# liruiluo/VLA-Adapter

Hardware: AMD Instinct MI355X
Metric: fine-tune samples/sec (224px img + 32-tok prompt), adapter-only, fwd+bwd+AdamW (higher is better)
Workload: dtype bf16

## Files before the change

### vla_adapter_amd/csrc/elementwise.hip

```cpp
#include "gemm_epilogue.h"
#include <type_traits>

namespace {

inline unsigned nblk(long long n, int per) { return (unsigned)((n + per - 1) / per); }

__global__ void im2col_kernel(const void* __restrict__ px, bf16_t* __restrict__ out, int B, int Ctot, int c0, int H,
                              int W, int P, int ldo, int f32in) {
  const int gw = W / P, gh = H / P, KK = 3 * P * P;
  const long long total = (long long)B * gh * gw * ldo;
  for (long long i = (long long)blockIdx.x * blockDim.x + threadIdx.x; i < total; i += (long long)gridDim.x * blockDim.x) {
    const int col = i % ldo;
    const long long prow = i / ldo;
    float v = 0.f;
    if (col < KK) {
      const int c = col / (P * P), rem = col - c * P * P, py = rem / P, pxx = rem - py * P;
      const int pw = prow % gw, ph = (prow / gw) % gh, b = prow / ((long long)gw * gh);
      const long long src = (((long long)b * Ctot + c0 + c) * H + ph * P + py) * W + pw * P + pxx;
      v = f32in ? ((const float*)px)[src] : bf2f(((const bf16_t*)px)[src]);
    }
    out[i] = f2bf(v);
  }
}

__global__ void action_mask_kernel(const long long* __restrict__ labels, int* __restrict__ qidx, int* __restrict__ pos,
                                   int* __restrict__ count, int B, int L, int shift) {
  const int b = blockIdx.x, lane = threadIdx.x;
  const long long* row = labels + (long long)b * L + shift;
  const int n = L - shift;
  int base = 0;
  for (int j0 = 0; j0 < n; j0 += 64) {
    const int j = j0 + lane;
    const bool sel = j < n && row[j] != -100 && row[j] > 151386;
    const unsigned long long bal = __ballot(sel);
    const int k = base + __popcll(bal & ((1ull << lane) - 1ull));
    if (j < n) qidx[(long long)b * n + j] = sel ? k : -1;
    if (sel && k < 64) pos[b * 64 + k] = j;
    base += __popcll(bal);
  }
  if (lane == 0) count[b] = base;
  for (int k = base + lane; k < 64; k += 64) pos[b * 64 + k] = -1;
}

__global__ void embed_splice_kernel(const long long* __restrict__ ids, const unsigned char* __restrict__ am,
                                    const int* __restrict__ qidx, const bf16_t* __restrict__ table,
                                    const bf16_t* __restrict__ aq, bf16_t* __restrict__ out,
                                    unsigned char* __restrict__ mm, int B, int L, int Np, int D, int vocab) {
  const int S = L + Np;
  const int lane = threadIdx.x & 63;
  const long long r = (long long)blockIdx.x * 4 + (threadIdx.x >> 6);
  if (r >= (long long)B * S) return;
  const int b = r / S, s = r - (long long)b * S;
  if (s >= 1 && s <= Np) {
    if (lane == 0 && mm) mm[r] = 1;
    return;
  }
  const int j = s == 0 ? 0 : s - Np;
  const int qi = qidx[(long long)b * L + j];
  long long id = ids[(long long)b * L + j];
  if (id < 0 || id >= vocab) id = 0;
  const bf16_t* src = qi >= 0 ? aq + (long long)min(qi, 63) * D : table + id * D;
  bf16_t* dst = out + r * D;
  for (int e = lane * 8; e < D; e += 512) *reinterpret_cast<uint4*>(dst + e) = *reinterpret_cast<const uint4*>(src + e);
  if (lane == 0 && mm) mm[r] = am ? (am[(long long)b * L + j] != 0) : 1;
}

__global__ void action_query_grad_kernel(const bf16_t* __restrict__ dx, const int* __restrict__ pos, float* __restrict__ dq,
                                         int B, int S, int Np, int D, int row0) {
  const int k = blockIdx.x;
  for (int d = threadIdx.x; d < D; d += blockDim.x) {
    float a = 0.f;
    for (int b = 0; b < B; ++b) {
      const int j = pos[b * 64 + k];
      if (j < 0) continue;
      const int s = (j == 0 ? 0 : Np + j) - row0;
      if (s < 0) continue;
      a += bf2f(dx[((long long)b * S + s) * D + d]);
    }
    dq[k * D + d] = a;
  }
}

__global__ void gather_rows_kernel(const bf16_t* __restrict__ in, const int* __restrict__ idx, bf16_t* __restrict__ out,
                                   int n, int D, int ldi, int ldo) {
  const int lane = threadIdx.x & 63;
  const long long r = (long long)blockIdx.x * 4 + (threadIdx.x >> 6);
  if (r >= n) return;
  const int s = idx[r];
  if (s == -2) return;
  for (int e = lane * 8; e < D; e += 512) {
    uint4 v = s >= 0 ? *reinterpret_cast<const uint4*>(in + (long long)s * ldi + e) : uint4{0, 0, 0, 0};
    *reinterpret_cast<uint4*>(out + r * ldo + e) = v;
  }
}

__global__ void scatter_add_rows_kernel(const bf16_t* __restrict__ in, const int* __restrict__ idx, bf16_t* __restrict__ out,
                                        int n, int D, int ldi, int ldo) {
  const int lane = threadIdx.x & 63;
  const long long r = (long long)blockIdx.x * 4 + (threadIdx.x >> 6);
  if (r >= n) return;
  const int s = idx[r];
  if (s < 0) return;
  for (int e = lane * 8; e < D; e += 512) {
    float a[8], c[8];
    unpack8(*reinterpret_cast<const uint4*>(in + r * ldi + e), a);
    unpack8(*reinterpret_cast<const uint4*>(out + (long long)s * ldo + e), c);
#pragma unroll
    for (int k = 0; k < 8; ++k) c[k] += a[k];
    *reinterpret_cast<uint4*>(out + (long long)s * ldo + e) = pack8(c);
  }
}

enum { EW_ADD = 0, EW_GELU_F = 1, EW_GELU_B = 2, EW_RELU_B = 3 };
template <int OP>
__global__ void ew_kernel(const bf16_t* __restrict__ a, const bf16_t* __restrict__ b, bf16_t* __restrict__ y, long long n8) {
  for (long long i = (long long)blockIdx.x * blockDim.x + threadIdx.x; i < n8; i += (long long)gridDim.x * blockDim.x) {
    float fa[8], fb[8] = {0, 0, 0, 0, 0, 0, 0, 0}, o[8];
    unpack8(reinterpret_cast<const uint4*>(a)[i], fa);
    if (OP != EW_GELU_F) unpack8(reinterpret_cast<const uint4*>(b)[i], fb);
#pragma unroll
    for (int k = 0; k < 8; ++k) {
      if (OP == EW_ADD) o[k] = fa[k] + fb[k];
      else if (OP == EW_GELU_F) o[k] = gelu_erf(fa[k]);
      else if (OP == EW_GELU_B) o[k] = fa[k] * gelu_erf_grad(fb[k]);
      else o[k] = fb[k] > 0.f ? fa[k] : 0.f;
    }
    reinterpret_cast<uint4*>(y)[i] = pack8(o);
  }
}

__global__ void swiglu_bwd_kernel(const bf16_t* __restrict__ dh, const bf16_t* __restrict__ gu, bf16_t* __restrict__ dgu,
                                  long long nchunks, int I) {
  const int cpr = I / 8;
  for (long long i = (long long)blockIdx.x * blockDim.x + threadIdx.x; i < nchunks; i += (long long)gridDim.x * blockDim.x) {
    const long long m = i / cpr;
    const int c = (int)(i - m * cpr) * 8;
    const long long go = m * 2 * I + (c >> 4) * 32 + (c & 15);
    float d[8], g[8], u[8], dg[8], du[8];
    unpack8(*reinterpret_cast<const uint4*>(dh + m * I + c), d);
    unpack8(*reinterpret_cast<const uint4*>(gu + go), g);
    unpack8(*reinterpret_cast<const uint4*>(gu + go + 16), u);
#pragma unroll
    for (int k = 0; k < 8; ++k) {
      const float sg = 1.f / (1.f + __expf(-g[k]));
      du[k] = d[k] * (g[k] * sg);
      dg[k] = d[k] * u[k] * silu_grad(g[k], sg);
    }
    *reinterpret_cast<uint4*>(dgu + go) = pack8(dg);
    *reinterpret_cast<uint4*>(dgu + go + 16) = pack8(du);
  }
}

__global__ __launch_bounds__(256) void transpose_kernel(const bf16_t* __restrict__ in, bf16_t* __restrict__ out, int rows,
                                                        int cols, int ldi, int ldo, long long s_in, long long s_out) {
  __shared__ bf16_t t[64][66];
  const bf16_t* ib = in + (long long)blockIdx.z * s_in;
  bf16_t* ob = out + (long long)blockIdx.z * s_out;
  const int r0 = blockIdx.y * 64, c0 = blockIdx.x * 64;
  const int tx = threadIdx.x & 63, ty = threadIdx.x >> 6;
  for (int r = ty; r < 64; r += 4)
    t[r][tx] = (r0 + r < rows && c0 + tx < cols) ? ib[(long long)(r0 + r) * ldi + c0 + tx] : (bf16_t)0;
  __syncthreads();
  for (int c = ty; c < 64; c += 4)
    if (c0 + c < cols && r0 + tx < rows) ob[(long long)(c0 + c) * ldo + r0 + tx] = t[tx][c];
}

__global__ __launch_bounds__(256) void transpose_vec_kernel(const bf16_t* __restrict__ in, bf16_t* __restrict__ out, int rows,
                                                            int cols, int ldi, int ldo, long long s_in, long long s_out) {
  __shared__ unsigned t32[64 * 33];
  const bf16_t* ib = in + (long long)blockIdx.z * s_in;
  bf16_t* ob = out + (long long)blockIdx.z * s_out;
  const int r0 = blockIdx.y * 64, c0 = blockIdx.x * 64;
  for (int i = threadIdx.x; i < 512; i += 256) {
    const int r = i >> 3, ch = i & 7;
    uint4 v = {0u, 0u, 0u, 0u};
    if (r0 + r < rows && c0 + ch * 8 < cols) v = *reinterpret_cast<const uint4*>(ib + (long long)(r0 + r) * ldi + c0 + ch * 8);
    unsigned* d = t32 + r * 33 + ch * 4;
    d[0] = v.x; d[1] = v.y; d[2] = v.z; d[3] = v.w;
  }
  __syncthreads();
  const bf16_t* t = reinterpret_cast<const bf16_t*>(t32);
  for (int i = threadIdx.x; i < 512; i += 256) {
    const int g = i & 7, c = i >> 3;
    if (c0 + c < cols && r0 + g * 8 < rows) {
      unsigned o[4];
#pragma unroll
      for (int k = 0; k < 4; ++k)
        o[k] = (unsigned)t[(g * 8 + 2 * k) * 66 + c] | ((unsigned)t[(g * 8 + 2 * k + 1) * 66 + c] << 16);
      *reinterpret_cast<uint4*>(ob + (long long)(c0 + c) * ldo + r0 + g * 8) = uint4{o[0], o[1], o[2], o[3]};
    }
  }
}

__global__ void colsum_kernel(const bf16_t* __restrict__ x, float* __restrict__ out, int rows, int cols, int ldx, long long s_x,
                              long long s_out) {
  const int c = blockIdx.x * 256 + threadIdx.x;
  if (c >= cols) return;
  x += (long long)blockIdx.z * s_x;
  out += (long long)blockIdx.z * s_out;
  float a = 0.f;
  for (int r = 0; r < rows; ++r) a += bf2f(x[(long long)r * ldx + c]);
  atomicAdd(out + c, a);
}

template <int LPR>
__global__ __launch_bounds__(CR_THREADS) void colsum_vec_kernel(const bf16_t* __restrict__ x, float* __restrict__ out, int rows, int cols,
                                                                int ldx, long long s_x, long long s_out) {
  __shared__ float sm[CR_THREADS / 64][64];
  const int c = CR<LPR>::col();
  x += (long long)blockIdx.z * s_x;
  out += (long long)blockIdx.z * s_out;
  float a[8] = {0, 0, 0, 0, 0, 0, 0, 0};
  if (c < cols)
    for (int r = CR<LPR>::row0(); r < rows; r += CR<LPR>::GROUPS) {
      float f[8];
      unpack8(*reinterpret_cast<const uint4*>(x + (long long)r * ldx + c), f);
#pragma unroll
      for (int k = 0; k < 8; ++k) a[k] += f[k];
    }
  CR<LPR>::add(a, out, cols, sm);
}

__global__ void cast_f32_bf16_kernel(const float* __restrict__ x, bf16_t* __restrict__ y, long long n) {
  for (long long i = (long long)blockIdx.x * blockDim.x + threadIdx.x; i < n; i += (long long)gridDim.x * blockDim.x) y[i] = f2bf(x[i]);
}
__global__ void cast_bf16_f32_kernel(const bf16_t* __restrict__ x, float* __restrict__ y, long long n) {
  for (long long i = (long long)blockIdx.x * blockDim.x + threadIdx.x; i < n; i += (long long)gridDim.x * blockDim.x) y[i] = bf2f(x[i]);
}

__global__ void rope_half_kernel(bf16_t* __restrict__ x, const float* __restrict__ ct, const float* __restrict__ st, long long rows,
                                 int S, int nheads, int dh, int ldx, float sign) {
  const int half = dh / 2;
  const long long total = rows * nheads * half;
// ... 130 lines not shown
template <bool CLIP>
__global__ void adamw_vec8_kernel(uint4* __restrict__ p, const void* __restrict__ g, uint4* __restrict__ m, uint4* __restrict__ v,
                                  long long n8, float decay, float omb1, float beta2, float omb2, float bc2_sqrt, float eps,
                                  float neg_step, int g_f32, float gscale, const float* __restrict__ coef) {
  const float c = CLIP ? *coef : 1.f;
  for (long long i = (long long)blockIdx.x * blockDim.x + threadIdx.x; i < n8; i += (long long)gridDim.x * blockDim.x) {
    const uint4 pv = p[i], mv = m[i], vv = v[i];
    float gr[8];
    adamw_grad8(g, i, g_f32, gscale, gr);
    if (CLIP) {
#pragma unroll
      for (int k = 0; k < 8; ++k) gr[k] = rbf(gr[k] * c);
    }
    const unsigned pw[4] = {pv.x, pv.y, pv.z, pv.w}, mw[4] = {mv.x, mv.y, mv.z, mv.w}, vw[4] = {vv.x, vv.y, vv.z, vv.w};
    unsigned po[4], mo[4], vo[4];
#pragma unroll
    for (int k = 0; k < 4; ++k) {
      float p0 = bf_lo(pw[k]), p1 = bf_hi(pw[k]);
      float m0 = bf_lo(mw[k]), m1 = bf_hi(mw[k]);
      float v0 = bf_lo(vw[k]), v1 = bf_hi(vw[k]);
      adamw_one(p0, gr[2 * k], m0, v0, decay, omb1, beta2, omb2, bc2_sqrt, eps, neg_step);
      adamw_one(p1, gr[2 * k + 1], m1, v1, decay, omb1, beta2, omb2, bc2_sqrt, eps, neg_step);
      po[k] = pack2(p0, p1); mo[k] = pack2(m0, m1); vo[k] = pack2(v0, v1);
    }
    p[i] = uint4{po[0], po[1], po[2], po[3]};
    m[i] = uint4{mo[0], mo[1], mo[2], mo[3]};
    v[i] = uint4{vo[0], vo[1], vo[2], vo[3]};
  }
}

constexpr int GRAD_SSQ_ITERS = 8;
constexpr long long GRAD_SSQ_CHUNK = 256LL * 8 * GRAD_SSQ_ITERS;
template <bool F32>
__global__ __launch_bounds__(256) void grad_sumsq_kernel(const void* __restrict__ g, long long n, float gscale, float* __restrict__ slots) {
  typedef typename std::conditional<F32, float, bf16_t>::type T;
  __shared__ float red[4];
  const long long c0 = (long long)blockIdx.x * GRAD_SSQ_CHUNK;
  const int cnt = (int)min(GRAD_SSQ_CHUNK, n - c0), tid = threadIdx.x;
  const T* base = (const T*)g + c0;
  const int head = min(cnt, (int)(((16 - ((uintptr_t)base & 15)) & 15) / sizeof(T)));
  const int nv = (cnt - head) / 8, tail0 = head + nv * 8;
  const T* body = base + head;
  float acc = 0.f, gr[8];
  if (nv == 256 * GRAD_SSQ_ITERS) {
    float x[GRAD_SSQ_ITERS][8];
#pragma unroll
    for (int it = 0; it < GRAD_SSQ_ITERS; ++it) adamw_grad8(body, it * 256 + tid, F32, gscale, x[it]);
#pragma unroll
    for (int it = 0; it < GRAD_SSQ_ITERS; ++it)
#pragma unroll
      for (int k = 0; k < 8; ++k) acc = __builtin_fmaf(x[it][k], x[it][k], acc);
  } else {
    for (int j = tid; j < nv; j += 256) {
      adamw_grad8(body, j, F32, gscale, gr);
#pragma unroll
      for (int k = 0; k < 8; ++k) acc = __builtin_fmaf(gr[k], gr[k], acc);
    }
  }
  if (tid < head) {
    const float x = adamw_grad<F32>(F32 ? ((const float*)base)[tid] : bf2f(((const bf16_t*)base)[tid]), gscale);
    acc = __builtin_fmaf(x, x, acc);
  }
  if (tid < cnt - tail0) {
    const float x = adamw_grad<F32>(F32 ? ((const float*)base)[tail0 + tid] : bf2f(((const bf16_t*)base)[tail0 + tid]), gscale);
    acc = __builtin_fmaf(x, x, acc);
  }
  acc = wave_sum(acc);
  if ((tid & 63) == 0) red[tid >> 6] = acc;
  __syncthreads();
  if (tid == 0) slots[blockIdx.x] = ((red[0] + red[1]) + red[2]) + red[3];
}

__global__ __launch_bounds__(256) void grad_norm_finalise_kernel(const float* __restrict__ slots, long long n_slots, float max_norm,
                                                                 float* __restrict__ out) {
  __shared__ double red[256];
  const int tid = threadIdx.x;
  double s = 0.0;
  for (long long i = tid; i < n_slots; i += 256) s += (double)slots[i];
  red[tid] = s;
  __syncthreads();
  for (int o = 128; o > 0; o >>= 1) {
    if (tid < o) red[tid] += red[tid + o];
    __syncthreads();
  }
  if (tid == 0) {
    const float total = (float)sqrt(red[0]);
    const float c = (1.f / (total + 1e-6f)) * max_norm;
    out[0] = total;
    out[1] = c > 1.f ? 1.f : c;
  }
}

}

#define GRID1D(n, per) dim3(min(nblk((n), (per)), 8192u))

__global__ void image_normalize_kernel(const unsigned char* __restrict__ img, void* __restrict__ out, int B, int H, int W, int Ctot,
                                       int c0, float m0, float m1, float m2, float s0, float s1, float s2, int out_f32) {
  const long long total = (long long)B * 3 * H * W;
  for (long long i = (long long)blockIdx.x * blockDim.x + threadIdx.x; i < total; i += (long long)gridDim.x * blockDim.x) {
    const int x = (int)(i % W);
    const int y = (int)((i / W) % H);
    const int c = (int)((i / ((long long)W * H)) % 3);
    const long long b = i / ((long long)3 * W * H);
    const float t = (float)img[((b * H + y) * W + x) * 3 + c] / 255.0f;
    const float v = (t - (c == 0 ? m0 : c == 1 ? m1 : m2)) / (c == 0 ? s0 : c == 1 ? s1 : s2);
    const long long o = ((b * Ctot + c0 + c) * H + y) * W + x;
    if (out_f32) reinterpret_cast<float*>(out)[o] = v;
    else reinterpret_cast<bf16_t*>(out)[o] = f2bf(v);
  }
}

__global__ void action_tokenize_kernel(const float* __restrict__ act, const double* __restrict__ bins, long long* __restrict__ ids,
                                       long long n, int nbins, float lo, float hi, long long tokenizer_len) {
  const long long i = (long long)blockIdx.x * blockDim.x + threadIdx.x;
  if (i >= n) return;
  ids[i] = action_token_id(act[i], bins, nbins, lo, hi, tokenizer_len);
}

extern "C" int vla_im2col_patch(void* stream, const void* pixels, void* cols, int B, int Ctot, int c0, int H, int W, int P,
                                int ldo, int px_f32) {
  VLA_REQUIRE(pixels && cols && B > 0 && P > 0 && H % P == 0 && W % P == 0, "im2col: bad shape");
  VLA_REQUIRE(c0 >= 0 && c0 + 3 <= Ctot && ldo >= 3 * P * P, "im2col: channel window / ldo");
  const long long total = (long long)B * (H / P) * (W / P) * ldo;
  hipLaunchKernelGGL(im2col_kernel, GRID1D(total, 256), dim3(256), 0, (hipStream_t)stream, pixels, (bf16_t*)cols, B, Ctot, c0,
                     H, W, P, ldo, px_f32);
  VLA_CHECK_LAUNCH("im2col");
  return VLA_OK;
}

extern "C" int vla_action_mask(void* stream, const long long* labels, int* qidx, int* pos, int* count, int B, int L, int shift) {
  VLA_REQUIRE(labels && qidx && pos && count && B > 0 && L > shift && (shift == 0 || shift == 1), "action_mask: bad args");
  hipLaunchKernelGGL(action_mask_kernel, dim3(B), dim3(64), 0, (hipStream_t)stream, labels, qidx, pos, count, B, L, shift);
  VLA_CHECK_LAUNCH("action_mask");
  return VLA_OK;
}

extern "C" int vla_embed_splice(void* stream, const long long* ids, const unsigned char* attn_mask, const int* qidx,
                                const void* table, const void* action_queries, void* out, unsigned char* mm_mask, int B,
                                int L, int Np, int D, int vocab) {
  VLA_REQUIRE(ids && qidx && table && action_queries && out && B > 0 && L > 0 && Np >= 0 && D % 8 == 0 && vocab > 0,
              "embed_splice: bad args");
  VLA_REQUIRE(((((uintptr_t)table) | ((uintptr_t)action_queries) | ((uintptr_t)out)) & 15) == 0, "embed_splice: 16-B aligned table / action_queries / out");
  const long long rows = (long long)B * (L + Np);
  hipLaunchKernelGGL(embed_splice_kernel, dim3(nblk(rows, 4)), dim3(256), 0, (hipStream_t)stream, ids, attn_mask, qidx,
                     (const bf16_t*)table, (const bf16_t*)action_queries, (bf16_t*)out, mm_mask, B, L, Np, D, vocab);
  VLA_CHECK_LAUNCH("embed_splice");
  return VLA_OK;
}

extern "C" int vla_action_query_grad(void* stream, const void* dx, const int* pos, float* dq, int B, int S, int Np, int D,
                                     int row0) {
  VLA_REQUIRE(dx && pos && dq && B > 0 && S > 0 && S + row0 > Np && D > 0 && row0 >= 0, "action_query_grad: bad args");
  hipLaunchKernelGGL(action_query_grad_kernel, dim3(64), dim3(256), 0, (hipStream_t)stream, (const bf16_t*)dx, pos, dq, B, S, Np, D, row0);
  VLA_CHECK_LAUNCH("action_query_grad");
  return VLA_OK;
}

extern "C" int vla_gather_rows(void* stream, const void* in, const int* idx, void* out, int n, int D, int ldi, int ldo) {
  VLA_REQUIRE(in && idx && out && n > 0 && D % 8 == 0 && ldi % 8 == 0 && ldo % 8 == 0, "gather_rows: bad args");
  VLA_REQUIRE(((((uintptr_t)in) | ((uintptr_t)out)) & 15) == 0, "gather_rows: 16-B aligned in / out");
  hipLaunchKernelGGL(gather_rows_kernel, dim3(nblk(n, 4)), dim3(256), 0, (hipStream_t)stream, (const bf16_t*)in, idx, (bf16_t*)out, n, D, ldi, ldo);
  VLA_CHECK_LAUNCH("gather_rows");
  return VLA_OK;
}

extern "C" int vla_scatter_add_rows(void* stream, const void* in, const int* idx, void* out, int n, int D, int ldi, int ldo) {
  VLA_REQUIRE(in && idx && out && n > 0 && D % 8 == 0 && ldi % 8 == 0 && ldo % 8 == 0, "scatter_add_rows: bad args");
  VLA_REQUIRE(((((uintptr_t)in) | ((uintptr_t)out)) & 15) == 0, "scatter_add_rows: 16-B aligned in / out");
  hipLaunchKernelGGL(scatter_add_rows_kernel, dim3(nblk(n, 4)), dim3(256), 0, (hipStream_t)stream, (const bf16_t*)in, idx, (bf16_t*)out, n, D, ldi, ldo);
  VLA_CHECK_LAUNCH("scatter_add_rows");
  return VLA_OK;
}

#define EW_ENTRY(NAME, OP, NEEDB)                                                                                  \
  extern "C" int NAME(void* stream, const void* a, const void* b, void* y, long long n) {                           \
    VLA_REQUIRE(a && y && (!(NEEDB) || b) && n > 0 && n % 8 == 0, #NAME ": null / n%8");                              \
    VLA_REQUIRE(((((uintptr_t)a) | ((uintptr_t)b) | ((uintptr_t)y)) & 15) == 0, #NAME ": 16-B aligned tensors");     \
    hipLaunchKernelGGL(ew_kernel<OP>, GRID1D(n / 8, 256), dim3(256), 0, (hipStream_t)stream, (const bf16_t*)a,     \
                       (const bf16_t*)b, (bf16_t*)y, n / 8);                                                       \
    VLA_CHECK_LAUNCH(#NAME);                                                                                       \
    return VLA_OK;                                                                                                 \
  }
EW_ENTRY(vla_add_bf16, EW_ADD, 1)
EW_ENTRY(vla_gelu_bwd, EW_GELU_B, 1)
EW_ENTRY(vla_relu_bwd, EW_RELU_B, 1)
extern "C" int vla_gelu_fwd(void* stream, const void* x, void* y, long long n) {
  VLA_REQUIRE(x && y && n > 0 && n % 8 == 0, "gelu_fwd: null / n%8");
  VLA_REQUIRE(((((uintptr_t)x) | ((uintptr_t)y)) & 15) == 0, "gelu_fwd: 16-B aligned tensors");
  hipLaunchKernelGGL(ew_kernel<EW_GELU_F>, GRID1D(n / 8, 256), dim3(256), 0, (hipStream_t)stream, (const bf16_t*)x,
                     (const bf16_t*)nullptr, (bf16_t*)y, n / 8);
  VLA_CHECK_LAUNCH("gelu_fwd");
  return VLA_OK;
}

extern "C" int vla_swiglu_bwd(void* stream, const void* dh, const void* gu, void* dgu, int M, int I) {
  VLA_REQUIRE(dh && gu && dgu && M > 0 && I > 0 && I % 16 == 0, "swiglu_bwd: I%16");
  VLA_REQUIRE(((((uintptr_t)dh) | ((uintptr_t)gu) | ((uintptr_t)dgu)) & 15) == 0, "swiglu_bwd: 16-B aligned tensors");
  const long long nch = (long long)M * (I / 8);
  hipLaunchKernelGGL(swiglu_bwd_kernel, GRID1D(nch, 256), dim3(256), 0, (hipStream_t)stream, (const bf16_t*)dh, (const bf16_t*)gu, (bf16_t*)dgu, nch, I);
  VLA_CHECK_LAUNCH("swiglu_bwd");
  return VLA_OK;
}

extern "C" int vla_transpose_bf16(void* stream, const void* in, void* out, int rows, int cols, int ldi, int ldo, int batch,
                                  long long s_in, long long s_out) {
  VLA_REQUIRE(in && out && rows > 0 && cols > 0 && ldi >= cols && ldo >= rows && batch > 0, "transpose: bad args");
  dim3 grid((cols + 63) / 64, (rows + 63) / 64, batch);
  const bool vec = rows % 8 == 0 && cols % 8 == 0 && ldi % 8 == 0 && ldo % 8 == 0 && s_in % 8 == 0 && s_out % 8 == 0 &&
                   ((((uintptr_t)in) | ((uintptr_t)out)) & 15) == 0;
  if (vec)
    hipLaunchKernelGGL(transpose_vec_kernel, grid, dim3(256), 0, (hipStream_t)stream, (const bf16_t*)in, (bf16_t*)out, rows, cols, ldi, ldo, s_in, s_out);
  else
    hipLaunchKernelGGL(transpose_kernel, grid, dim3(256), 0, (hipStream_t)stream, (const bf16_t*)in, (bf16_t*)out, rows, cols, ldi, ldo, s_in, s_out);
  VLA_CHECK_LAUNCH("transpose");
  return VLA_OK;
}

extern "C" int vla_colsum_bf16(void* stream, const void* x, float* out, int rows, int cols, int ldx, int batch, long long s_x,
                               long long s_out) {
  VLA_REQUIRE(x && out && rows > 0 && cols > 0 && ldx >= cols && batch > 0, "colsum: bad args");
  if (cols % 8 == 0 && ldx % 8 == 0 && s_x % 8 == 0 && ((uintptr_t)x & 15) == 0) {
    CR_LAUNCH(colsum_vec_kernel, rows, cols, batch, stream, (const bf16_t*)x, out, rows, cols, ldx, s_x, s_out);
    VLA_CHECK_LAUNCH("colsum");
    return VLA_OK;
  }
  hipLaunchKernelGGL(colsum_kernel, dim3((cols + 255) / 256, 1, batch), dim3(256), 0, (hipStream_t)stream, (const bf16_t*)x, out, rows,
                     cols, ldx, s_x, s_out);
  VLA_CHECK_LAUNCH("colsum");
  return VLA_OK;
}

extern "C" int vla_cast_f32_bf16(void* stream, const float* x, void* y, long long n) {
  VLA_REQUIRE(x && y && n > 0, "cast: bad args");
  hipLaunchKernelGGL(cast_f32_bf16_kernel, GRID1D(n, 256), dim3(256), 0, (hipStream_t)stream, x, (bf16_t*)y, n);
  VLA_CHECK_LAUNCH("cast_f32_bf16");
  return VLA_OK;
}
extern "C" int vla_cast_bf16_f32(void* stream, const void* x, float* y, long long n) {
  VLA_REQUIRE(x && y && n > 0, "cast: bad args");
  hipLaunchKernelGGL(cast_bf16_f32_kernel, GRID1D(n, 256), dim3(256), 0, (hipStream_t)stream, (const bf16_t*)x, y, n);
  VLA_CHECK_LAUNCH("cast_bf16_f32");
  return VLA_OK;
}

extern "C" int vla_rope_half(void* stream, void* x, const float* cos_t, const float* sin_t, int rows, int S, int nheads, int dh,
                             int ldx, int sign) {
  VLA_REQUIRE(x && cos_t && sin_t && rows > 0 && S > 0 && nheads > 0 && dh % 2 == 0 && ldx >= nheads * dh, "rope_half: bad args");
  const long long total = (long long)rows * nheads * (dh / 2);
  hipLaunchKernelGGL(rope_half_kernel, GRID1D(total, 256), dim3(256), 0, (hipStream_t)stream, (bf16_t*)x, cos_t, sin_t, (long long)rows, S, nheads, dh, ldx, sign >= 0 ? 1.f : -1.f);
  VLA_CHECK_LAUNCH("rope_half");
  return VLA_OK;
}

extern "C" int vla_rope_interleaved(void* stream, void* x, const float* cos_t, const float* sin_t, int rows, int T, int nheads,
                                    int dh, int ldx, int mode) {
  VLA_REQUIRE(x && cos_t && sin_t && rows > 0 && T > 0 && nheads > 0 && dh % 2 == 0 && ldx >= nheads * dh, "rope_interleaved: bad args");
  const long long total = (long long)rows * nheads * (dh / 2);
  if (dh % 8 == 0 && ldx % 8 == 0 && (((uintptr_t)x | (uintptr_t)cos_t | (uintptr_t)sin_t) & 15) == 0) {
    const long long tv = (long long)rows * (nheads * dh / 8);
    hipLaunchKernelGGL(rope_inter_vec_kernel, GRID1D(tv, 256), dim3(256), 0, (hipStream_t)stream, (bf16_t*)x, cos_t, sin_t, (int)rows, T, nheads, dh, ldx, mode);
  } else
  hipLaunchKernelGGL(rope_inter_kernel, GRID1D(total, 256), dim3(256), 0, (hipStream_t)stream, (bf16_t*)x, cos_t, sin_t, (long long)rows, T, nheads, dh, ldx, mode);
  VLA_CHECK_LAUNCH("rope_interleaved");
  return VLA_OK;
}

extern "C" int vla_l1_loss(void* stream, const void* pred, const void* target, float* loss3, void* dpred, int B, int C, int Da,
                           float gscale) {
  VLA_REQUIRE(pred && target && loss3 && B > 0 && C > 0 && Da > 0, "l1_loss: bad args");
  hipLaunchKernelGGL(l1_loss_kernel, dim3(1), dim3(256), 0, (hipStream_t)stream, (const bf16_t*)pred, (const bf16_t*)target, loss3, (bf16_t*)dpred, B, C, Da, gscale);
  VLA_CHECK_LAUNCH("l1_loss");
  return VLA_OK;
}

static int adamw_launch(void* stream, void* p, const void* g, void* m, void* v, long long n, double lr, double beta1, double beta2,
                        double eps, double wd, int step, int g_f32, float gscale, const float* coef) {
  VLA_REQUIRE(p && g && m && v && n > 0 && step >= 1, "adamw: bad args");
  const double bc1 = 1.0 - pow(beta1, step), bc2 = 1.0 - pow(beta2, step);
  const float decay = (float)(1.0 - lr * wd);
  const float omb1 = (float)(1.0 - beta1), omb2 = (float)(1.0 - beta2);
  const float neg_step = (float)(-(lr / bc1));
  const float gs = gscale == 0.f ? 1.f : gscale;
  const bool aligned = ((((uintptr_t)p) | ((uintptr_t)g) | ((uintptr_t)m) | ((uintptr_t)v)) & 15) == 0;
  const long long n8 = aligned ? n / 8 : 0, done = n8 * 8;
  if (n8 > 0)
    hipLaunchKernelGGL(coef ? adamw_vec8_kernel<true> : adamw_vec8_kernel<false>, GRID1D(n8, 256), dim3(256), 0, (hipStream_t)stream,
                       (uint4*)p, g, (uint4*)m, (uint4*)v, n8, decay, omb1, (float)beta2, omb2, (float)sqrt(bc2), (float)eps, neg_step,
                       g_f32, gs, coef);
  if (done < n)
    hipLaunchKernelGGL(coef ? adamw_kernel<true> : adamw_kernel<false>, GRID1D(n - done, 256), dim3(256), 0, (hipStream_t)stream,
                       (bf16_t*)p + done, g_f32 ? (const void*)((const float*)g + done) : (const void*)((const bf16_t*)g + done),
                       (bf16_t*)m + done, (bf16_t*)v + done, n - done, decay, omb1, (float)beta2, omb2, (float)sqrt(bc2), (float)eps,
                       neg_step, g_f32, gs, coef);
  VLA_CHECK_LAUNCH("adamw");
  return VLA_OK;
}

extern "C" int vla_adamw_bf16(void* stream, void* p, const void* g, void* m, void* v, long long n, double lr, double beta1,
                              double beta2, double eps, double wd, int step, int g_f32, float gscale) {
  return adamw_launch(stream, p, g, m, v, n, lr, beta1, beta2, eps, wd, step, g_f32, gscale, nullptr);
}

extern "C" int vla_adamw_clipped_bf16(void* stream, void* p, const void* g, void* m, void* v, long long n, double lr, double beta1,
                                      double beta2, double eps, double wd, int step, int g_f32, float gscale, const float* coef) {
  VLA_REQUIRE(coef, "adamw_clipped: null coefficient");
  return adamw_launch(stream, p, g, m, v, n, lr, beta1, beta2, eps, wd, step, g_f32, gscale, coef);
}

extern "C" long long vla_grad_sumsq_slots(long long n) { return n > 0 ? (n + GRAD_SSQ_CHUNK - 1) / GRAD_SSQ_CHUNK : 0; }

extern "C" int vla_grad_sumsq(void* stream, const void* g, long long n, int g_f32, float gscale, float* slots) {
  VLA_REQUIRE(g && slots && n > 0, "grad_sumsq: bad args");
  VLA_REQUIRE(((uintptr_t)g & (g_f32 ? 3 : 1)) == 0 && ((uintptr_t)slots & 3) == 0, "grad_sumsq: misaligned pointer");
  const long long nb = vla_grad_sumsq_slots(n);
  VLA_REQUIRE(nb <= 0x7fffffffLL, "grad_sumsq: slice too long");
  const float gs = gscale == 0.f ? 1.f : gscale;
  hipLaunchKernelGGL(g_f32 ? grad_sumsq_kernel<true> : grad_sumsq_kernel<false>, dim3((unsigned)nb), dim3(256), 0, (hipStream_t)stream, g, n, gs, slots);
  VLA_CHECK_LAUNCH("grad_sumsq");
  return VLA_OK;
}

extern "C" int vla_grad_norm_finalise(void* stream, const float* slots, long long n_slots, float max_norm, float* out2) {
  VLA_REQUIRE(slots && out2 && n_slots > 0 && max_norm > 0.f, "grad_norm_finalise: bad args");
  hipLaunchKernelGGL(grad_norm_finalise_kernel, dim3(1), dim3(256), 0, (hipStream_t)stream, slots, n_slots, max_norm, out2);
  VLA_CHECK_LAUNCH("grad_norm_finalise");
  return VLA_OK;
}

extern "C" int vla_image_normalize_u8(void* stream, const void* img, void* out, int B, int H, int W, int Ctot, int c0,
                                      const float* mean3, const float* std3, int out_f32) {
  VLA_REQUIRE(img && out && mean3 && std3 && B > 0 && H > 0 && W > 0 && c0 >= 0 && c0 + 3 <= Ctot, "image_normalize: bad args");
  VLA_REQUIRE(std3[0] != 0.f && std3[1] != 0.f && std3[2] != 0.f, "image_normalize: zero std");
  const long long total = (long long)B * 3 * H * W;
  hipLaunchKernelGGL(image_normalize_kernel, GRID1D(total, 256), dim3(256), 0, (hipStream_t)stream, (const unsigned char*)img, out, B,
                     H, W, Ctot, c0, mean3[0], mean3[1], mean3[2], std3[0], std3[1], std3[2], out_f32);
  VLA_CHECK_LAUNCH("image_normalize");
  return VLA_OK;
}

extern "C" int vla_action_tokenize(void* stream, const float* actions, const double* bins, long long* ids, long long n, int nbins,
                                   float lo, float hi, long long tokenizer_len) {
  VLA_REQUIRE(actions && bins && ids && n > 0 && nbins > 1 && lo < hi, "action_tokenize: bad args");
  hipLaunchKernelGGL(action_tokenize_kernel, dim3((unsigned)((n + 255) / 256)), dim3(256), 0, (hipStream_t)stream, actions, bins, ids, n,
                     nbins, lo, hi, tokenizer_len);
  VLA_CHECK_LAUNCH("action_tokenize");
  return VLA_OK;
}


template <typename TS, typename TD>
__global__ void copy2d_kernel(const TS* __restrict__ src, TD* __restrict__ dst, long long rows, int cols, long long ld_src, long long ld_dst,
                              int src_mod, int d_group, long long d_group_stride) {
  const long long total = rows * cols;
  for (long long i = (long long)blockIdx.x * blockDim.x + threadIdx.x; i < total; i += (long long)gridDim.x * blockDim.x) {
    const long long r = i / cols;
    const int c = (int)(i - r * cols);
    const long long rs = src_mod > 0 ? r % src_mod : r;
    const long long ro = d_group > 0 ? (r / d_group) * d_group_stride + (r % d_group) * ld_dst : r * ld_dst;
    float v;
    if constexpr (sizeof(TS) == 2) v = bf2f(src[rs * ld_src + c]); else v = src[rs * ld_src + c];
    if constexpr (sizeof(TD) == 2) dst[ro + c] = f2bf(v); else dst[ro + c] = v;
  }
}

__global__ void quant_fp8_rows_kernel(const bf16_t* __restrict__ x, unsigned char* __restrict__ q, float* __restrict__ scale, int rows, int cols,
                                      long long ldx, long long ldq) {
  const int lane = threadIdx.x & 63, row = blockIdx.x * (blockDim.x >> 6) + (threadIdx.x >> 6);
  if (row >= rows) return;
  const bf16_t* xr = x + (long long)row * ldx;
  float amax = 0.f;
  for (int c = lane * 8; c < cols; c += 512) {
    const uint4 v = *reinterpret_cast<const uint4*>(xr + c);
    const unsigned w[4] = {v.x, v.y, v.z, v.w};
#pragma unroll
    for (int k = 0; k < 4; ++k) amax = fmaxf(amax, fmaxf(fabsf(bf_lo(w[k])), fabsf(bf_hi(w[k]))));
  }
  amax = wave_max(amax);
  const float inv = amax > 0.f ? __fdiv_rn(448.f, amax) : 1.f;
  if (lane == 0) scale[row] = amax > 0.f ? __fdiv_rn(amax, 448.f) : 1.f;
  unsigned char* qr = q + (long long)row * ldq;
  for (int c = lane * 8; c < cols; c += 512) {
    const uint4 v = *reinterpret_cast<const uint4*>(xr + c);
    const unsigned w[4] = {v.x, v.y, v.z, v.w};
    int lo = 0, hi = 0;
    lo = __builtin_amdgcn_cvt_pk_fp8_f32(bf_lo(w[0]) * inv, bf_hi(w[0]) * inv, lo, false);
    lo = __builtin_amdgcn_cvt_pk_fp8_f32(bf_lo(w[1]) * inv, bf_hi(w[1]) * inv, lo, true);
    hi = __builtin_amdgcn_cvt_pk_fp8_f32(bf_lo(w[2]) * inv, bf_hi(w[2]) * inv, hi, false);
    hi = __builtin_amdgcn_cvt_pk_fp8_f32(bf_lo(w[3]) * inv, bf_hi(w[3]) * inv, hi, true);
    *reinterpret_cast<uint2*>(qr + c) = uint2{(unsigned)lo, (unsigned)hi};
  }
}

extern "C" int vla_quant_fp8_rows(void* stream, const void* x, void* q, float* scale, int rows, int cols, int ldx, int ldq) {
  VLA_REQUIRE(x && q && scale && rows > 0 && cols > 0 && cols % 8 == 0 && ldx % 8 == 0 && ldx >= cols && ldq >= cols && ldq % 16 == 0 &&
                  ((((uintptr_t)x) | ((uintptr_t)q)) & 15) == 0,
              "quant_fp8_rows: cols % 8, ldx % 8, ldq % 16, 16-B aligned pointers");
  hipLaunchKernelGGL(quant_fp8_rows_kernel, dim3((rows + 3) / 4), dim3(256), 0, (hipStream_t)stream, (const bf16_t*)x, (unsigned char*)q, scale, rows,
                     cols, (long long)ldx, (long long)ldq);
  VLA_CHECK_LAUNCH("quant_fp8_rows");
  return VLA_OK;
}

__global__ void copy2d_vec_kernel(const uint4* __restrict__ src, uint4* __restrict__ dst, long long rows, long long cols16, long long ld_src16,
                                  long long ld_dst16) {
  const long long total = rows * cols16;
  for (long long i = (long long)blockIdx.x * blockDim.x + threadIdx.x; i < total; i += (long long)gridDim.x * blockDim.x) {
    const long long r = i / cols16, c = i - r * cols16;
    dst[r * ld_dst16 + c] = src[r * ld_src16 + c];
  }
}

extern "C" int vla_copy2d(void* stream, const void* src, void* dst, long long rows, int cols, long long ld_src, long long ld_dst,
                          int src_dtype, int dst_dtype, int src_mod, int d_group, long long d_group_stride) {
  VLA_REQUIRE(src && dst && rows > 0 && cols > 0 && src_mod >= 0 && d_group >= 0, "copy2d: bad args");
  VLA_REQUIRE((src_dtype == 0 || src_dtype == 1) && (dst_dtype == 0 || dst_dtype == 1), "copy2d: dtype 0 (bf16) / 1 (f32)");
  hipStream_t st = (hipStream_t)stream;
  const int esz = src_dtype == 0 ? 2 : 4, per16 = 16 / esz;
  if (src_dtype == dst_dtype && src_mod == 0 && d_group == 0 && cols % per16 == 0 && ld_src % per16 == 0 && ld_dst % per16 == 0 &&
      ((((uintptr_t)src) | ((uintptr_t)dst)) & 15) == 0) {
    const long long c16 = cols / per16;
    hipLaunchKernelGGL(copy2d_vec_kernel, GRID1D(rows * c16, 256), dim3(256), 0, st, (const uint4*)src, (uint4*)dst, rows, c16, ld_src / per16,
                       ld_dst / per16);
    VLA_CHECK_LAUNCH("copy2d");
    return VLA_OK;
  }
  const dim3 g = GRID1D(rows * cols, 256);
#define CP(TS, TD) hipLaunchKernelGGL((copy2d_kernel<TS, TD>), g, dim3(256), 0, st, (const TS*)src, (TD*)dst, rows, cols, ld_src, ld_dst, src_mod, d_group, d_group_stride)
  if (src_dtype == 0 && dst_dtype == 0) CP(bf16_t, bf16_t);
  else if (src_dtype == 1 && dst_dtype == 0) CP(float, bf16_t);
  else if (src_dtype == 0 && dst_dtype == 1) CP(bf16_t, float);
  else CP(float, float);
#undef CP
  VLA_CHECK_LAUNCH("copy2d");
  return VLA_OK;
}

__global__ void fill_zero_kernel(uint4* __restrict__ p16, long long n16, unsigned char* __restrict__ tail, int ntail) {
  const long long i0 = (long long)blockIdx.x * blockDim.x + threadIdx.x;
  for (long long i = i0; i < n16; i += (long long)gridDim.x * blockDim.x) p16[i] = uint4{0, 0, 0, 0};
  if (i0 < ntail) tail[i0] = 0;
}

extern "C" int vla_fill_zero(void* stream, void* ptr, long long nbytes) {
  VLA_REQUIRE(ptr && nbytes > 0 && ((uintptr_t)ptr & 15) == 0, "fill_zero: null / empty / not 16-B aligned");
  const long long n16 = nbytes / 16;
  hipLaunchKernelGGL(fill_zero_kernel, GRID1D(n16 > 0 ? n16 : 1, 256), dim3(256), 0, (hipStream_t)stream, (uint4*)ptr, n16,
                     (unsigned char*)ptr + n16 * 16, (int)(nbytes - n16 * 16));
  VLA_CHECK_LAUNCH("fill_zero");
  return VLA_OK;
}

__device__ __forceinline__ unsigned long long drop_hash(unsigned long long seed, unsigned long long idx) { return splitmix64_key(seed, idx); }

template <bool ADD>
__global__ void dropout_kernel(const bf16_t* __restrict__ x, bf16_t* __restrict__ y, long long rows, int cols, long long ldx, long long ldy,
                               unsigned thr, float scale, unsigned long long seed, const int* __restrict__ step) {
  const int cpr = cols >> 3;
  const long long total = rows * cpr;
  const unsigned long long sd = seed + (unsigned long long)(step ? *step : 0) * 0xD1B54A32D192ED03ull;
  for (long long i = (long long)blockIdx.x * blockDim.x + threadIdx.x; i < total; i += (long long)gridDim.x * blockDim.x) {
    const long long r = i / cpr;
    const int c = (int)(i - r * cpr) * 8;
    const unsigned long long h0 = drop_hash(sd, 2ull * (unsigned long long)i), h1 = drop_hash(sd, 2ull * (unsigned long long)i + 1);
    const uint4 xv = *reinterpret_cast<const uint4*>(x + r * ldx + c);
    const unsigned xw[4] = {xv.x, xv.y, xv.z, xv.w};
    uint4 yv = uint4{0, 0, 0, 0};
    if (ADD) yv = *reinterpret_cast<const uint4*>(y + r * ldy + c);
    unsigned yw[4] = {yv.x, yv.y, yv.z, yv.w};
#pragma unroll
    for (int k = 0; k < 4; ++k) {
      const unsigned long long h = k < 2 ? h0 : h1;
      const bool k0 = ((unsigned)(h >> (32 * (k & 1))) & 0xffffu) >= thr, k1 = ((unsigned)(h >> (32 * (k & 1) + 16)) & 0xffffu) >= thr;
      const float a = k0 ? rbf(bf_lo(xw[k]) * scale) : 0.f, b = k1 ? rbf(bf_hi(xw[k]) * scale) : 0.f;
      if (ADD) yw[k] = pack2(bf_lo(yw[k]) + a, bf_hi(yw[k]) + b);
      else yw[k] = pack2(a, b);
    }
    *reinterpret_cast<uint4*>(y + r * ldy + c) = uint4{yw[0], yw[1], yw[2], yw[3]};
  }
}

static int dropout_launch(bool add, void* stream, const void* x, void* y, long long rows, int cols, long long ldx, long long ldy, float p,
                          unsigned long long seed, const int* step) {
  VLA_REQUIRE(x && y && rows > 0 && cols > 0 && cols % 8 == 0 && ldx % 8 == 0 && ldy % 8 == 0 && (((uintptr_t)x | (uintptr_t)y) & 15) == 0,
              "dropout: null / empty / cols, row strides must be multiples of 8 and the tensors 16-B aligned");
  VLA_REQUIRE(p >= 0.f && p < 1.f, "dropout: p in [0, 1)");
  const unsigned thr = (unsigned)(p * 65536.f + 0.5f);
  const float scale = 1.f / (1.f - p);
  const long long total = rows * (cols / 8);
  if (add) hipLaunchKernelGGL(dropout_kernel<true>, GRID1D(total, 256), dim3(256), 0, (hipStream_t)stream, (const bf16_t*)x, (bf16_t*)y, rows, cols, ldx, ldy, thr, scale, seed, step);
  else hipLaunchKernelGGL(dropout_kernel<false>, GRID1D(total, 256), dim3(256), 0, (hipStream_t)stream, (const bf16_t*)x, (bf16_t*)y, rows, cols, ldx, ldy, thr, scale, seed, step);
  VLA_CHECK_LAUNCH("dropout");
  return VLA_OK;
}

extern "C" int vla_dropout_bf16(void* stream, const void* x, void* y, long long rows, int cols, long long ldx, long long ldy, float p,
                                unsigned long long seed, const int* step) {
  return dropout_launch(false, stream, x, y, rows, cols, ldx, ldy, p, seed, step);
}

extern "C" int vla_dropout_bwd_add_bf16(void* stream, const void* u, void* dx, long long rows, int cols, long long ldu, long long lddx, float p,
                                        unsigned long long seed, const int* step) {
  return dropout_launch(true, stream, u, dx, rows, cols, ldu, lddx, p, seed, step);
}

__global__ void inc_i32_kernel(int* p) { if (threadIdx.x == 0 && blockIdx.x == 0) *p += 1; }

extern "C" int vla_inc_i32(void* stream, int* ptr) {
  VLA_REQUIRE(ptr, "inc_i32: null");
  hipLaunchKernelGGL(inc_i32_kernel, dim3(1), dim3(64), 0, (hipStream_t)stream, ptr);
  VLA_CHECK_LAUNCH("inc_i32");
  return VLA_OK;
}

__global__ void head_index_prep_kernel(const int* __restrict__ pos1, const int* __restrict__ pos0, const int* __restrict__ cnt0,
                                       int* __restrict__ gather, int* __restrict__ scatter, float* __restrict__ guard,
                                       int B, int S, int Np, int row0) {
  const int i = blockIdx.x * blockDim.x + threadIdx.x;
  if (i < B * 65) {
    const int b = i / 65, k = i - b * 65;
    if (k == 64) {
      gather[i] = -2;
      scatter[i] = -1;
    } else {
      const int p = pos1[b * 64 + k];
      gather[i] = b * S + Np + p;
      const int loc = Np + p - row0;
      scatter[i] = (loc >= 0 && p >= 0) ? b * (S - row0) + loc : -1;
    }
  }
  if (i == 0 && guard) {
    bool bad = false;
    for (int b = 0; b < B; ++b) bad |= (row0 > 0) && ((cnt0[b] > 0 ? pos0[b * 64] + Np : 0) < row0);
    *guard = bad ? __int_as_float(0x7fc00000) : 0.f;
  }
}

extern "C" int vla_head_index_prep(void* stream, const int* pos1, const int* pos0, const int* cnt0, int* gather, int* scatter,
                                   float* guard, int B, int S, int Np, int row0) {
  VLA_REQUIRE(pos1 && pos0 && cnt0 && gather && scatter && B > 0 && S > row0 && row0 >= 0, "head_index_prep: bad args");
  hipLaunchKernelGGL(head_index_prep_kernel, dim3(nblk((long long)B * 65, 256)), dim3(256), 0, (hipStream_t)stream, pos1, pos0, cnt0, gather,
                     scatter, guard, B, S, Np, row0);
  VLA_CHECK_LAUNCH("head_index_prep");
  return VLA_OK;
}

__global__ void add_scalar_f32_kernel(float* __restrict__ x, const float* __restrict__ s, int n) {
  const int i = blockIdx.x * blockDim.x + threadIdx.x;
  if (i < n) x[i] += *s;
}

extern "C" int vla_add_scalar_f32(void* stream, float* x, const float* s, int n) {
  VLA_REQUIRE(x && s && n > 0, "add_scalar_f32: bad args");
  hipLaunchKernelGGL(add_scalar_f32_kernel, dim3(nblk(n, 256)), dim3(256), 0, (hipStream_t)stream, x, s, n);
  VLA_CHECK_LAUNCH("add_scalar_f32");
  return VLA_OK;
}


__global__ void embed_grad_kernel(const bf16_t* __restrict__ dx, const long long* __restrict__ ids, const int* __restrict__ qidx,
                                  bf16_t* __restrict__ gtable, int B, int L, int Np, int D, int vocab) {
  const int t = blockIdx.x, n = B * L;
  if (qidx[t] >= 0) return;
  long long id = ids[t];
  if (id < 0 || id >= vocab) id = 0;
  __shared__ int first;
  if (threadIdx.x == 0) {
    int f = 1;
    for (int u = 0; u < t && f; ++u) {
      long long iu = ids[u];
      if (iu < 0 || iu >= vocab) iu = 0;
      if (qidx[u] < 0 && iu == id) f = 0;
    }
    first = f;
  }
  __syncthreads();
// ... 394 lines not shown
```

### vla_adapter_amd/engine.py

```python
from __future__ import annotations

import contextlib
import math
import os
from dataclasses import dataclass, field
from typing import Dict, List, Optional, Tuple

import torch

from . import ops, schedule
from .ops import ACT_GELU, ACT_GELU_TANH, ACT_NONE, ACT_RELU, ACT_SWIGLU, BF16
from .schedule import Segment, capture_graph, chunks, turnaround_chunks

NUM_TOKENS = 64
IGNORE_INDEX = -100


def rup(n: int, m: int) -> int:
    return (n + m - 1) // m * m


def copy_flat(dst: torch.Tensor, src: torch.Tensor):
    n = src.numel()
    ops.copy2d(src, dst, 1, n, n, n)
# ... 1143 lines not shown
                self._query_grad()

        return (schedule.pipeline_forward(head, fch, llm_fwd, lambda: (llm.HS, self.pos1, batch["proprio"], self.Np, noise), turn_around,
                                          refresh=True)
                + schedule.pipeline_backward(head, fch, llm_bwd, lambda: self._dHS)
                + [Segment("H", head.bwd_end, None, ("end", 0))])

    def _stream_of(self, name: str, main):
        return main if name == "M" else self.side if name == "H" else self._vstreams[int(name[1:])]

    def _cap_stream(self, name: str):
        return self._cap_main if name == "M" else self._stream_of(name, None)

    def _fwd_bwd(self, batch, noise, vision: bool = True):
        self.executed_steps += 1
        if vision:
            self._vision(batch)
        torch.cuda.current_stream().wait_event(schedule.run(self._segments(batch, noise), self._stream_of)[("end", 0)])
        return self._loss3

    def capture(self, batch: Dict[str, torch.Tensor], noise: Optional[torch.Tensor] = None, warmup: int = 2,
                conservative_rows: bool = False, row0: Optional[int] = None):
        self._ensure_streams()
        self._static_batch, self._static_noise = batch, noise
        self._row0 = None
        self._vision_and_embed(batch)
        self._row0 = self.live_row0()
        if conservative_rows and not self.full_llm_backward:
            self._row0 = min(self._row0, (self.cfg.n_patches + 1) // 32 * 32)
        if row0 is not None:
            assert 0 <= int(row0) < self.S and int(row0) % 32 == 0, f"row0 {row0}: a multiple of 32 inside the sequence"
            self._row0 = int(row0)
        for _ in range(warmup):
            self.head.dirty = True
            self._fwd_bwd(batch, noise)
        torch.cuda.synchronize()
        self.head.dirty = True
        self._next_px = batch["pixel_values"].clone()
        self._px_stage = batch["pixel_values"].clone()
        self._g_vis = capture_graph(lambda: self._vision(dict(batch, pixel_values=self._px_stage)), torch.cuda.graph_pool_handle(),
                                    self.vis_stream)
        self._vis_ev = None
        self._segs = self._segments(batch, noise)
        self._graphs = schedule.capture(self._segs, {}, self._cap_stream)
        torch.cuda.synchronize()
        self._pending_lr = None
        m_fwd = [k for k, sg in enumerate(self._segs) if sg.stream == "M" and sg.signal is not None and sg.signal[0] == "f"]
        self._vis_after = m_fwd[min(len(m_fwd) - 1, max(0, int(os.environ.get("VLA_VIS_AFTER", len(m_fwd) - 4))))]
        assert self._segs[self._vis_after].signal is not None
        self._launch_vision()

    def stage_next_pixels(self, pixel_values: torch.Tensor):
        if self._px_copied is not None:
            torch.cuda.current_stream().wait_event(self._px_copied)
        self._next_px.copy_(pixel_values)

    def _launch_vision(self, after_event=None):
        V, cur = self.vis_stream, torch.cuda.current_stream()
        if after_event is not None:
            V.wait_event(after_event)
        else:
            V.wait_stream(cur)
        tl = self._timeline
        with torch.cuda.stream(V):
            if tl is not None:
                t0 = torch.cuda.Event(enable_timing=True)
                t0.record(V)
            copy_flat(self._px_stage, self._next_px)
            self._px_copied = torch.cuda.Event()
            self._px_copied.record(V)
            self._g_vis.replay()
            self._vis_ev = torch.cuda.Event(enable_timing=tl is not None)
            self._vis_ev.record(V)
            if tl is not None:
                tl.append(("V", -1, t0, self._vis_ev))

    def train_step_pipelined(self, batch, lr: float, noise=None):
        self._ensure_streams()
        loss3 = self._fwd_bwd(batch, noise)
        if self.reducer is not None:
            self.reducer.reduce_async(self.head.P.grad, 0, None)
        self.optimizer_step(lr)
        return loss3

    def train_step_graphed(self, lr: float):
        cur = torch.cuda.current_stream()
        self.executed_steps += 1
        self.flush(join=False)
        cur.wait_event(self._vis_ev)
        def after(k, seg, ev):
            if k == self._vis_after:
                self._launch_vision(ev)
        self._h_end = schedule.run(self._segs, self._stream_of, self._graphs, after=after,
                                   timeline=self._timeline)[("end", 0)]
        cur.wait_event(self._px_copied)
        if self.ga > 1:
            cur.wait_event(self._h_end)
            if not self._accum.fold():
                return self._loss3
            self._h_end = torch.cuda.Event()
            self._h_end.record(cur)
        if self.reducer is not None:
            aq_off = self.head.P.offsets["action_queries"][0]
            ev_aq = self.reducer.reduce_async(self.head.P.grad, aq_off, None)
            ev_head = self.reducer.reduce_async(self.head.P.grad, 0, aq_off, after_event=self._h_end)
            self._reduced = (ev_aq, ev_head)
        self._pending_lr = lr
        return self._loss3

    def flush(self, join: bool = True):
        if self._pending_lr is None:
            return
        lr, self._pending_lr = self._pending_lr, None
        self._apply_update(lr, two_stream=True, join=join)

    def _apply_update(self, lr: float, beta1=0.9, beta2=0.999, eps=1e-8, wd=0.01, *, two_stream: bool, join: bool):
        cur, P, clip = torch.cuda.current_stream(), self.head.P, self._clip
        hs = self.side if two_stream else cur
        aq_off = P.offsets["action_queries"][0]
        assert aq_off + rup(math.prod(P.offsets["action_queries"][1]), 8) == P.numel, "action_queries must close the flat buffer"
        self.step_count += 1
        gscale = 1.0
        if self.reducer is not None:
            ev_aq, ev_head = self._reduced or (None, None)
            if ev_aq is not None and ev_head is not None:
                cur.wait_event(ev_aq)
                hs.wait_event(ev_head)
                self.reducer.joined()
            else:
                self.reducer.wait(*((cur, hs) if two_stream else (cur,)))
            self._reduced = None
            gscale = self.reducer.grad_scale
        if two_stream and self.ga > 1:
            hs.wait_event(self._h_end)
        if clip is not None:
            r_head, r_aq = self._clip_ranges()
            head_summed, finalised = self._clip_events
            clip.begin([r_head, r_aq])
            with torch.cuda.stream(hs):
                clip.sumsq(*r_head, gscale)
                head_summed.record(hs)
            clip.sumsq(*r_aq, gscale)
            cur.wait_event(head_summed)
            clip.finalise()
            finalised.record(cur)
            hs.wait_event(finalised)

        def adam(sl):
            args = (self.step_count, lr, beta1, beta2, eps, wd)
            if clip is None:
                ops.adamw_(P.data[sl], P.grad[sl], P.m[sl], P.v[sl], *args, gscale=gscale)
            else:
                ops.adamw_clipped_(P.data[sl], P.grad[sl], P.m[sl], P.v[sl], clip.coef, *args, gscale=gscale)
        with torch.cuda.stream(hs):
            adam(slice(None, aq_off))
            side_done = torch.cuda.Event()
            side_done.record()
        adam(slice(aq_off, None))
        if join:
            cur.wait_event(side_done)
        self.head.dirty = True

    def begin_validation(self):
        self.flush()
        if self._vis_ev is not None:
            torch.cuda.current_stream().wait_event(self._vis_ev)
        self.head.refresh_forward_operands()

    def end_validation(self):
        if self._g_vis is not None:
            self._launch_vision()

    def val_forward(self, batch: Dict[str, torch.Tensor], noise: Optional[torch.Tensor] = None) -> torch.Tensor:
        pred = self._val_pred = self.forward(batch, noise)
        return ops.l1_loss(pred, self._to_bf16(batch["actions"]), want_grad=False)[0]

    @property
    def val_pred(self) -> torch.Tensor:
        return self._val_pred.view(self.B, self.cfg.chunk, self.cfg.action_dim)

    def val_step_graphed(self, batch: Dict[str, torch.Tensor], noise: Optional[torch.Tensor] = None) -> torch.Tensor:
        self._ensure_streams()

        def make():
            segs = self._predict_segments(batch, noise, loss_of=batch["actions"])
            return schedule.capture(segs, {}, self._cap_stream), segs

        def replay(graphs, segs):
            self.head.refresh_forward_operands()
            torch.cuda.current_stream().wait_event(schedule.run(segs, self._stream_of, graphs)[("end", 0)])
        return schedule.captured_validation(self, batch, noise, make, replay)
```

Before: 1318.

## Vectorize action-query grad and grouped copy2d; reorder AdamW launches across streams

```diff
diff --git a/vla_adapter_amd/csrc/elementwise.hip b/vla_adapter_amd/csrc/elementwise.hip
--- a/vla_adapter_amd/csrc/elementwise.hip
+++ b/vla_adapter_amd/csrc/elementwise.hip
@@ -79,6 +79,39 @@
     }
     dq[k * D + d] = a;
   }
+}
+
+constexpr int AQ_WIN = 16;
+__global__ __launch_bounds__(64) void action_query_grad_vec_kernel(const bf16_t* __restrict__ dx, const int* __restrict__ pos,
+                                                                   float* __restrict__ dq, int B, int S, int Np, int D, int row0) {
+  const int k = blockIdx.x, d = (blockIdx.y * 64 + threadIdx.x) * 8;
+  if (d >= D) return;
+  float a[8] = {0.f, 0.f, 0.f, 0.f, 0.f, 0.f, 0.f, 0.f};
+  for (int b0 = 0; b0 < B; b0 += AQ_WIN) {
+    int s[AQ_WIN];
+#pragma unroll
+    for (int i = 0; i < AQ_WIN; ++i) {
+      const int j = b0 + i < B ? pos[(b0 + i) * 64 + k] : -1;
+      s[i] = j < 0 ? -1 : (j == 0 ? 0 : Np + j) - row0;
+    }
+    uint4 v[AQ_WIN];
+#pragma unroll
+    for (int i = 0; i < AQ_WIN; ++i)
+      v[i] = *reinterpret_cast<const uint4*>(dx + ((long long)min(b0 + i, B - 1) * S + max(s[i], 0)) * D + d);
+#pragma unroll
+    for (int i = 0; i < AQ_WIN; ++i) {
+      if (s[i] < 0) continue;
+      const unsigned w[4] = {v[i].x, v[i].y, v[i].z, v[i].w};
+#pragma unroll
+      for (int e = 0; e < 4; ++e) {
+        a[2 * e] += bf_lo(w[e]);
+        a[2 * e + 1] += bf_hi(w[e]);
+      }
+    }
+  }
+  float4* o = reinterpret_cast<float4*>(dq + (long long)k * D + d);
+  o[0] = float4{a[0], a[1], a[2], a[3]};
+  o[1] = float4{a[4], a[5], a[6], a[7]};
 }
 
 __global__ void gather_rows_kernel(const bf16_t* __restrict__ in, const int* __restrict__ idx, bf16_t* __restrict__ out,
@@ -515,7 +548,11 @@
 extern "C" int vla_action_query_grad(void* stream, const void* dx, const int* pos, float* dq, int B, int S, int Np, int D,
                                      int row0) {
   VLA_REQUIRE(dx && pos && dq && B > 0 && S > 0 && S + row0 > Np && D > 0 && row0 >= 0, "action_query_grad: bad args");
-  hipLaunchKernelGGL(action_query_grad_kernel, dim3(64), dim3(256), 0, (hipStream_t)stream, (const bf16_t*)dx, pos, dq, B, S, Np, D, row0);
+  if (D % 8 == 0 && ((((uintptr_t)dx) | ((uintptr_t)dq)) & 15) == 0)
+    hipLaunchKernelGGL(action_query_grad_vec_kernel, dim3(64, (D / 8 + 63) / 64), dim3(64), 0, (hipStream_t)stream, (const bf16_t*)dx, pos, dq, B, S,
+                       Np, D, row0);
+  else
+    hipLaunchKernelGGL(action_query_grad_kernel, dim3(64), dim3(256), 0, (hipStream_t)stream, (const bf16_t*)dx, pos, dq, B, S, Np, D, row0);
   VLA_CHECK_LAUNCH("action_query_grad");
   return VLA_OK;
 }
@@ -774,17 +811,32 @@
   }
 }
 
+__global__ void copy2d_vec_group_kernel(const uint4* __restrict__ src, uint4* __restrict__ dst, long long rows, long long cols16, long long ld_src16,
+                                        long long ld_dst16, int src_mod, int d_group, long long d_group_stride16) {
+  const long long total = rows * cols16;
+  for (long long i = (long long)blockIdx.x * blockDim.x + threadIdx.x; i < total; i += (long long)gridDim.x * blockDim.x) {
+    const long long r = i / cols16, c = i - r * cols16;
+    const long long rs = src_mod > 0 ? r % src_mod : r;
+    const long long ro = d_group > 0 ? (r / d_group) * d_group_stride16 + (r % d_group) * ld_dst16 : r * ld_dst16;
+    dst[ro + c] = src[rs * ld_src16 + c];
+  }
+}
+
 extern "C" int vla_copy2d(void* stream, const void* src, void* dst, long long rows, int cols, long long ld_src, long long ld_dst,
                           int src_dtype, int dst_dtype, int src_mod, int d_group, long long d_group_stride) {
   VLA_REQUIRE(src && dst && rows > 0 && cols > 0 && src_mod >= 0 && d_group >= 0, "copy2d: bad args");
   VLA_REQUIRE((src_dtype == 0 || src_dtype == 1) && (dst_dtype == 0 || dst_dtype == 1), "copy2d: dtype 0 (bf16) / 1 (f32)");
   hipStream_t st = (hipStream_t)stream;
   const int esz = src_dtype == 0 ? 2 : 4, per16 = 16 / esz;
-  if (src_dtype == dst_dtype && src_mod == 0 && d_group == 0 && cols % per16 == 0 && ld_src % per16 == 0 && ld_dst % per16 == 0 &&
+  if (src_dtype == dst_dtype && cols % per16 == 0 && ld_src % per16 == 0 && ld_dst % per16 == 0 && (d_group == 0 || d_group_stride % per16 == 0) &&
       ((((uintptr_t)src) | ((uintptr_t)dst)) & 15) == 0) {
     const long long c16 = cols / per16;
-    hipLaunchKernelGGL(copy2d_vec_kernel, GRID1D(rows * c16, 256), dim3(256), 0, st, (const uint4*)src, (uint4*)dst, rows, c16, ld_src / per16,
-                       ld_dst / per16);
+    if (src_mod == 0 && d_group == 0)
+      hipLaunchKernelGGL(copy2d_vec_kernel, GRID1D(rows * c16, 256), dim3(256), 0, st, (const uint4*)src, (uint4*)dst, rows, c16, ld_src / per16,
+                         ld_dst / per16);
+    else
+      hipLaunchKernelGGL(copy2d_vec_group_kernel, GRID1D(rows * c16, 256), dim3(256), 0, st, (const uint4*)src, (uint4*)dst, rows, c16,
+                         ld_src / per16, ld_dst / per16, src_mod, d_group, d_group_stride / per16);
     VLA_CHECK_LAUNCH("copy2d");
     return VLA_OK;
   }
diff --git a/vla_adapter_amd/engine.py b/vla_adapter_amd/engine.py
--- a/vla_adapter_amd/engine.py
+++ b/vla_adapter_amd/engine.py
@@ -1319,11 +1319,11 @@
                 ops.adamw_(P.data[sl], P.grad[sl], P.m[sl], P.v[sl], *args, gscale=gscale)
             else:
                 ops.adamw_clipped_(P.data[sl], P.grad[sl], P.m[sl], P.v[sl], clip.coef, *args, gscale=gscale)
+        adam(slice(aq_off, None))
         with torch.cuda.stream(hs):
             adam(slice(None, aq_off))
             side_done = torch.cuda.Event()
             side_done.record()
-        adam(slice(aq_off, None))
         if join:
             cur.wait_event(side_done)
         self.head.dirty = True
```

After: 1318. About the same (-0.0%).
